# kongzhecn/OMG

Measured on NVIDIA H100. Metric: 1024^2 images/sec @30 steps, 2 concepts, higher is better.
Workload: dtype f16

## Files before the change

omg_b200/csrc/attn_tc.cu:

```cuda
#include <cuda_fp16.h>

#include <algorithm>
#include <math.h>
#include <stdlib.h>
#include <string.h>

#include "../../include/omg_b200.h"
#include "host_common.h"
#include "ptx.cuh"
#include "wgmma.cuh"

namespace omg {

constexpr int ATT_BQ = 128;
constexpr int ATT_BKV = 64;
constexpr int ATT_D = 64;
constexpr int ATT_Q_BYTES = ATT_BQ * ATT_D * 2;
constexpr int ATT_K_BYTES = ATT_BKV * ATT_D * 2;
constexpr int ATT_KV_STAGES = 4;
constexpr int ATT_THREADS = 256;
constexpr int ATT_SMEM = 1024 + ATT_Q_BYTES + ATT_KV_STAGES * 2 * ATT_K_BYTES + 256;

struct alignas(64) AttnParams {
    CUtensorMap q_map, k_map, v_map;
    __half* out;
    int out_ld;
    long long out_bs;
    int n_q, n_kv, heads;
    int q_col0, k_col0, v_col0, out_col0;
    int n_items;
    int out_b[OMG_ATTN_MAX_ITEMS], q_b[OMG_ATTN_MAX_ITEMS], k_b[OMG_ATTN_MAX_ITEMS], v_b[OMG_ATTN_MAX_ITEMS];
    float scale_log2;
    float out_weight;
    int accumulate;
    int causal;
};

__global__ void __launch_bounds__(ATT_THREADS, 2) attn_tc_kernel(const __grid_constant__ AttnParams p) {
    extern __shared__ uint8_t smem_raw[];
    uint8_t* smem = reinterpret_cast<uint8_t*>((reinterpret_cast<uintptr_t>(smem_raw) + 1023) & ~uintptr_t(1023));
    uint8_t* q_smem = smem;
    uint8_t* kv_smem = q_smem + ATT_Q_BYTES;
    uint64_t* q_full = reinterpret_cast<uint64_t*>(kv_smem + ATT_KV_STAGES * 2 * ATT_K_BYTES);
    uint64_t* kv_full = q_full + 1;
    uint64_t* kv_empty = kv_full + ATT_KV_STAGES;

    const int warp = threadIdx.x >> 5;
    const int lane = threadIdx.x & 31;
    const int slab = blockIdx.x, head = blockIdx.y, item = blockIdx.z;
    const int nkv = (p.n_kv + ATT_BKV - 1) / ATT_BKV;

    const int kb = p.k_b[item], vb = p.v_b[item];
    auto load_kv = [&](int jb) {
        const int st = jb % ATT_KV_STAGES;
        mbar_wait_nocall(&kv_empty[st], ((jb / ATT_KV_STAGES) & 1) ^ 1);
        uint8_t* kd = kv_smem + st * 2 * ATT_K_BYTES;
        mbar_arrive_expect_tx(&kv_full[st], 2 * ATT_K_BYTES);
        tma_load_3d(kd, &p.k_map, &kv_full[st], p.k_col0 + head * ATT_D, jb * ATT_BKV, kb);
        tma_load_3d(kd + ATT_K_BYTES, &p.v_map, &kv_full[st], p.v_col0 + head * ATT_D, jb * ATT_BKV, vb);
    };
    if (threadIdx.x == 0) {
        tma_prefetch_desc(&p.q_map);
        tma_prefetch_desc(&p.k_map);
        tma_prefetch_desc(&p.v_map);
        mbar_init(q_full, 1);
        for (int i = 0; i < ATT_KV_STAGES; ++i) {
            mbar_init(&kv_full[i], 1);
            mbar_init(&kv_empty[i], 2);
        }
        fence_barrier_init();
    }
    __syncthreads();
    griddep_launch_dependents();
    griddep_wait();
    if (threadIdx.x == 0) {
        mbar_arrive_expect_tx(q_full, ATT_Q_BYTES);
        tma_load_3d(q_smem, &p.q_map, q_full, p.q_col0 + head * ATT_D, slab * ATT_BQ, p.q_b[item]);
        for (int jb = 0; jb < ATT_KV_STAGES && jb < nkv; ++jb) load_kv(jb);
    }

    const int wg = warp >> 2, wi = warp & 3;
    const int g = lane >> 2, c = lane & 3;
    const int qrow0 = slab * ATT_BQ + wg * 64 + wi * 16 + g;
    const uint32_t q_addr = smem_u32(q_smem) + wg * (64 * 128);
    float o[32];
#pragma unroll
    for (int i = 0; i < 32; ++i) o[i] = 0.f;
    float m[2] = {-INFINITY, -INFINITY}, l[2] = {0.f, 0.f};
    mbar_wait_nocall(q_full, 0);
    for (int j = 0; j < nkv; ++j) {
        const int st = j % ATT_KV_STAGES;
        mbar_wait_nocall(&kv_full[st], (j / ATT_KV_STAGES) & 1);
        const uint32_t k_addr = smem_u32(kv_smem + st * 2 * ATT_K_BYTES);
        float s[32];
#pragma unroll
        for (int i = 0; i < 32; ++i) s[i] = 0.f;
        wgmma_fence();
#pragma unroll
        for (int k = 0; k < ATT_D / 16; ++k)
            wgmma_ss_n64(s, gmma_desc_sw128(q_addr + k * 32, 1024, 16), gmma_desc_sw128(k_addr + k * 32, 1024, 16), 1u);
        wgmma_commit();
        if (threadIdx.x == 0 && j >= 1 && j - 1 + ATT_KV_STAGES < nkv) load_kv(j - 1 + ATT_KV_STAGES);
        __syncwarp();
        wgmma_wait<0>();
        reg_fence(s);
        const int key0 = j * ATT_BKV + 2 * c;
        if ((j + 1) * ATT_BKV > p.n_kv || p.causal) {
#pragma unroll
            for (int J = 0; J < 8; ++J)
#pragma unroll
                for (int h = 0; h < 2; ++h)
#pragma unroll
                    for (int e = 0; e < 2; ++e) {
                        const int key = key0 + 8 * J + e;
                        if (key >= p.n_kv || (p.causal && key > qrow0 + 8 * h)) s[4 * J + 2 * h + e] = -INFINITY;
                    }
        }
        float mx[2] = {-INFINITY, -INFINITY};
#pragma unroll
        for (int J = 0; J < 8; ++J)
#pragma unroll
            for (int h = 0; h < 2; ++h) mx[h] = fmaxf(mx[h], fmaxf(s[4 * J + 2 * h], s[4 * J + 2 * h + 1]));
        float corr[2];
#pragma unroll
        for (int h = 0; h < 2; ++h) {
            mx[h] = fmaxf(mx[h], __shfl_xor_sync(0xffffffffu, mx[h], 1));
            mx[h] = fmaxf(mx[h], __shfl_xor_sync(0xffffffffu, mx[h], 2));
            const float m_new = fmaxf(m[h], mx[h] * p.scale_log2);
            corr[h] = fast_exp2(m[h] - m_new);
            m[h] = m_new;
            l[h] *= corr[h];
        }
#pragma unroll
        for (int J = 0; J < 8; ++J)
#pragma unroll
            for (int h = 0; h < 2; ++h) {
                o[4 * J + 2 * h] *= corr[h];
                o[4 * J + 2 * h + 1] *= corr[h];
            }
        uint32_t pa[4][4];
#pragma unroll
        for (int kk = 0; kk < 4; ++kk)
#pragma unroll
            for (int t = 0; t < 4; ++t) {
                const int h = t & 1, i0 = 8 * kk + 4 * (t >> 1) + 2 * h;
                const float p0 = fast_exp2(fmaf(s[i0], p.scale_log2, -m[h]));
                const float p1 = fast_exp2(fmaf(s[i0 + 1], p.scale_log2, -m[h]));
                l[h] += p0 + p1;
                pa[kk][t] = pack_half2(p0, p1);
            }
        const uint32_t v_addr = k_addr + ATT_K_BYTES;
        wgmma_fence();
#pragma unroll
        for (int kk = 0; kk < 4; ++kk)
            wgmma_rs_n64_tb(o, pa[kk], gmma_desc_sw128(v_addr + kk * 2048, 1024, 1024), 1u);
        wgmma_commit();
        wgmma_wait<0>();
        reg_fence(o);
        if ((threadIdx.x & 127) == 0) mbar_arrive(&kv_empty[st]);
    }

#pragma unroll
    for (int h = 0; h < 2; ++h) {
        l[h] += __shfl_xor_sync(0xffffffffu, l[h], 1);
        l[h] += __shfl_xor_sync(0xffffffffu, l[h], 2);
        const int qrow = qrow0 + 8 * h;
        if (qrow < p.n_q) {
            const float inv = p.out_weight / l[h];
            __half* op = p.out + (long long)p.out_b[item] * p.out_bs + (long long)qrow * p.out_ld + p.out_col0 +
                         head * ATT_D + 2 * c;
#pragma unroll
            for (int J = 0; J < 8; ++J) {
                float v0 = o[4 * J + 2 * h] * inv, v1 = o[4 * J + 2 * h + 1] * inv;
                __half2* dst = reinterpret_cast<__half2*>(op + 8 * J);
                if (p.accumulate) {
                    const float2 f = __half22float2(*dst);
                    v0 += f.x;
                    v1 += f.y;
                }
                *dst = __floats2half2_rn(v0, v1);
            }
        }
    }
}

static int make_attn_map(CUtensorMap* m, const void* ptr, int cols, int ld, int tokens, long long bs, int nb,
                         uint32_t box_rows) {
    const uint64_t dims[3] = {(uint64_t)cols, (uint64_t)tokens, (uint64_t)nb};
    const uint64_t strides[3] = {1, (uint64_t)ld, (uint64_t)bs};
    const uint32_t box[3] = {64, box_rows, 1};
    return make_tmap(m, CU_TENSOR_MAP_DATA_TYPE_FLOAT16, ptr, 3, dims, strides, box, CU_TENSOR_MAP_SWIZZLE_128B);
}

}

using namespace omg;

static int attention_impl(const omg_attn_desc* d, void* stream_) {
    cudaStream_t stream = reinterpret_cast<cudaStream_t>(stream_);
    OMG_CHECK(d != nullptr, "omg_attention: null descriptor");
    OMG_CHECK(d->head_dim == 64, "omg_attention: head_dim %d unsupported (SDXL uses 64)", d->head_dim);
    OMG_CHECK(d->n_items >= 1 && d->n_items <= OMG_ATTN_MAX_ITEMS, "omg_attention: n_items=%d out of range",
              d->n_items);
    OMG_CHECK(d->n_q >= 1 && d->n_kv >= 1 && d->heads >= 1, "omg_attention: empty problem");
    OMG_CHECK(d->q && d->k && d->v && d->out, "omg_attention: null pointer");
    OMG_CHECK(d->out_ld % 8 == 0 && d->out_col0 % 8 == 0 && d->out_bs % 8 == 0,
              "omg_attention: output must be 16 B aligned per row");
    if (check_head_windows("omg_attention", d->heads, d->head_dim, {d->q_col0, d->k_col0, d->v_col0, d->out_col0},
                           {d->q_ld, d->k_ld, d->v_ld, d->out_ld}))
        return 1;
    OMG_CHECK(!d->causal || (d->n_kv <= 128 && d->n_q <= 128), "omg_attention: causal masking is available for sequences of <= 128 tokens");
    static bool configured = false;
    if (!configured) {
        OMG_CUDA(cudaFuncSetAttribute(attn_tc_kernel, cudaFuncAttributeMaxDynamicSharedMemorySize, ATT_SMEM));
        configured = true;
    }
    AttnParams p;
    memset(&p, 0, sizeof(p));
    int max_qb = 0, max_kb = 0, max_vb = 0;
    for (int i = 0; i < d->n_items; ++i) {
        p.out_b[i] = d->out_b[i];
        p.q_b[i] = d->q_b[i];
        p.k_b[i] = d->k_b[i];
        p.v_b[i] = d->v_b[i];
        max_qb = d->q_b[i] > max_qb ? d->q_b[i] : max_qb;
        max_kb = d->k_b[i] > max_kb ? d->k_b[i] : max_kb;
        max_vb = d->v_b[i] > max_vb ? d->v_b[i] : max_vb;
        OMG_CHECK(d->out_b[i] >= 0 && d->q_b[i] >= 0 && d->k_b[i] >= 0 && d->v_b[i] >= 0,
                  "omg_attention: negative batch index in item %d", i);
    }
    const int cols = d->heads * 64;
    if (make_attn_map(&p.q_map, d->q, d->q_col0 + cols, d->q_ld, d->n_q, d->q_bs, max_qb + 1, ATT_BQ)) return 1;
    if (make_attn_map(&p.k_map, d->k, d->k_col0 + cols, d->k_ld, d->n_kv, d->k_bs, max_kb + 1, ATT_BKV)) return 1;
    if (make_attn_map(&p.v_map, d->v, d->v_col0 + cols, d->v_ld, d->n_kv, d->v_bs, max_vb + 1, ATT_BKV)) return 1;
    p.out = static_cast<__half*>(d->out);
    p.out_ld = d->out_ld;
    p.out_bs = d->out_bs;
    p.n_q = d->n_q;
    p.n_kv = d->n_kv;
    p.heads = d->heads;
    p.q_col0 = d->q_col0;
    p.k_col0 = d->k_col0;
    p.v_col0 = d->v_col0;
    p.out_col0 = d->out_col0;
    p.n_items = d->n_items;
    p.scale_log2 = d->scale * 1.4426950408889634f;
    p.out_weight = d->out_weight;
    p.accumulate = d->accumulate;
    p.causal = d->causal;
    dim3 grid((d->n_q + ATT_BQ - 1) / ATT_BQ, d->heads, d->n_items);
    OMG_CUDA(launch_pdl(attn_tc_kernel, grid, dim3(ATT_THREADS), ATT_SMEM, stream, p));
    return check_launch("attn_tc_kernel");
}

extern "C" int omg_attention(const omg_attn_desc* d, void* stream_) {
    const int rc = attention_impl(d, stream_);
    if (rc == 0 && ::omg::plan_recording()) {
        const omg_attn_desc c = *d;
        ::omg::plan_note([c](void* s) { return attention_impl(&c, s); });
    }
    return rc;
}
```

Measured before the change: 0.2027.

## Restructure attention into persistent warp-specialized kernel with pingpong softmax overlap

Rewrites the flash attention kernel as a persistent, warp-specialized design. A producer warp issues TMA loads for Q (double-buffered) and K/V tiles, and two consumer warpgroups alternate wgmma issue through turn barriers. The QK^T of the next block overlaps with PV and softmax of the current one. It also enlarges the KV block to 128, rebalances registers with setmaxnreg, and computes part of the exponentials with a polynomial exp2 to offload the SFU. This adds scheduling complexity, a grid of at most one CTA per SM, and slight numeric differences from the polynomial exp.

```diff
diff --git a/omg_b200/csrc/attn_tc.cu b/omg_b200/csrc/attn_tc.cu
--- a/omg_b200/csrc/attn_tc.cu
+++ b/omg_b200/csrc/attn_tc.cu
@@ -13,13 +13,14 @@
 namespace omg {
 
 constexpr int ATT_BQ = 128;
-constexpr int ATT_BKV = 64;
+constexpr int ATT_BKV = 128;
 constexpr int ATT_D = 64;
 constexpr int ATT_Q_BYTES = ATT_BQ * ATT_D * 2;
 constexpr int ATT_K_BYTES = ATT_BKV * ATT_D * 2;
 constexpr int ATT_KV_STAGES = 4;
-constexpr int ATT_THREADS = 256;
-constexpr int ATT_SMEM = 1024 + ATT_Q_BYTES + ATT_KV_STAGES * 2 * ATT_K_BYTES + 256;
+constexpr int ATT_THREADS = 384;
+constexpr int ATT_SMEM = 1024 + 2 * ATT_Q_BYTES + ATT_KV_STAGES * 2 * ATT_K_BYTES + 256;
+constexpr int ATT_POLY8 = 1;
 
 struct alignas(64) AttnParams {
     CUtensorMap q_map, k_map, v_map;
@@ -29,6 +30,7 @@
     int n_q, n_kv, heads;
     int q_col0, k_col0, v_col0, out_col0;
     int n_items;
+    int n_qt, n_tiles;
     int out_b[OMG_ATTN_MAX_ITEMS], q_b[OMG_ATTN_MAX_ITEMS], k_b[OMG_ATTN_MAX_ITEMS], v_b[OMG_ATTN_MAX_ITEMS];
     float scale_log2;
     float out_weight;
@@ -36,34 +38,40 @@
     int causal;
 };
 
-__global__ void __launch_bounds__(ATT_THREADS, 2) attn_tc_kernel(const __grid_constant__ AttnParams p) {
+__device__ __forceinline__ float poly_exp2(float x) {
+    x = fmaxf(x, -126.f);
+    const float t = __fadd_rd(x, 12582912.f);
+    const float f = x - (t - 12582912.f);
+    const float p = fmaf(fmaf(fmaf(0.07802452892065048f, f, 0.22606714069843292f), f, 0.6958335638046265f), f,
+                         0.9999251961708069f);
+    return __uint_as_float(__float_as_uint(p) + (__float_as_uint(t) << 23));
+}
+
+__global__ void __launch_bounds__(ATT_THREADS, 1) attn_tc_kernel(const __grid_constant__ AttnParams p) {
     extern __shared__ uint8_t smem_raw[];
     uint8_t* smem = reinterpret_cast<uint8_t*>((reinterpret_cast<uintptr_t>(smem_raw) + 1023) & ~uintptr_t(1023));
     uint8_t* q_smem = smem;
-    uint8_t* kv_smem = q_smem + ATT_Q_BYTES;
+    uint8_t* kv_smem = q_smem + 2 * ATT_Q_BYTES;
     uint64_t* q_full = reinterpret_cast<uint64_t*>(kv_smem + ATT_KV_STAGES * 2 * ATT_K_BYTES);
-    uint64_t* kv_full = q_full + 1;
+    uint64_t* q_empty = q_full + 2;
+    uint64_t* kv_full = q_empty + 2;
     uint64_t* kv_empty = kv_full + ATT_KV_STAGES;
+    uint64_t* turn_bar = kv_empty + ATT_KV_STAGES;
 
     const int warp = threadIdx.x >> 5;
     const int lane = threadIdx.x & 31;
-    const int slab = blockIdx.x, head = blockIdx.y, item = blockIdx.z;
     const int nkv = (p.n_kv + ATT_BKV - 1) / ATT_BKV;
-
-    const int kb = p.k_b[item], vb = p.v_b[item];
-    auto load_kv = [&](int jb) {
-        const int st = jb % ATT_KV_STAGES;
-        mbar_wait_nocall(&kv_empty[st], ((jb / ATT_KV_STAGES) & 1) ^ 1);
-        uint8_t* kd = kv_smem + st * 2 * ATT_K_BYTES;
-        mbar_arrive_expect_tx(&kv_full[st], 2 * ATT_K_BYTES);
-        tma_load_3d(kd, &p.k_map, &kv_full[st], p.k_col0 + head * ATT_D, jb * ATT_BKV, kb);
-        tma_load_3d(kd + ATT_K_BYTES, &p.v_map, &kv_full[st], p.v_col0 + head * ATT_D, jb * ATT_BKV, vb);
-    };
-    if (threadIdx.x == 0) {
+    const int per_item = p.n_qt * p.heads;
+
+    if (warp == 8 && lane == 0) {
         tma_prefetch_desc(&p.q_map);
         tma_prefetch_desc(&p.k_map);
         tma_prefetch_desc(&p.v_map);
-        mbar_init(q_full, 1);
+        for (int i = 0; i < 2; ++i) {
+            mbar_init(&q_full[i], 1);
+            mbar_init(&q_empty[i], 2);
+            mbar_init(&turn_bar[i], 1);
+        }
         for (int i = 0; i < ATT_KV_STAGES; ++i) {
             mbar_init(&kv_full[i], 1);
             mbar_init(&kv_empty[i], 2);
@@ -73,112 +81,204 @@
     __syncthreads();
     griddep_launch_dependents();
     griddep_wait();
-    if (threadIdx.x == 0) {
-        mbar_arrive_expect_tx(q_full, ATT_Q_BYTES);
-        tma_load_3d(q_smem, &p.q_map, q_full, p.q_col0 + head * ATT_D, slab * ATT_BQ, p.q_b[item]);
-        for (int jb = 0; jb < ATT_KV_STAGES && jb < nkv; ++jb) load_kv(jb);
-    }
-
+
+    if (warp >= 8) {
+        asm volatile("setmaxnreg.dec.sync.aligned.u32 40;");
+        if (warp == 8 && lane == 0) {
+            int kv_i = 0;
+            for (int t = blockIdx.x, qi = 0; t < p.n_tiles; t += gridDim.x, ++qi) {
+                const int item = t / per_item, head = (t % per_item) / p.n_qt, qt = t % p.n_qt;
+                const int qb = qi & 1;
+                mbar_wait_nocall(&q_empty[qb], ((qi >> 1) & 1) ^ 1);
+                mbar_arrive_expect_tx(&q_full[qb], ATT_Q_BYTES);
+                tma_load_3d(q_smem + qb * ATT_Q_BYTES, &p.q_map, &q_full[qb], p.q_col0 + head * ATT_D, qt * ATT_BQ,
+                            p.q_b[item]);
+                const int kb = p.k_b[item], vb = p.v_b[item];
+                for (int jb = 0; jb < nkv; ++jb, ++kv_i) {
+                    const int st = kv_i % ATT_KV_STAGES;
+                    mbar_wait_nocall(&kv_empty[st], ((kv_i / ATT_KV_STAGES) & 1) ^ 1);
+                    uint8_t* kd = kv_smem + st * 2 * ATT_K_BYTES;
+                    mbar_arrive_expect_tx(&kv_full[st], 2 * ATT_K_BYTES);
+                    tma_load_3d(kd, &p.k_map, &kv_full[st], p.k_col0 + head * ATT_D, jb * ATT_BKV, kb);
+                    tma_load_3d(kd + ATT_K_BYTES, &p.v_map, &kv_full[st], p.v_col0 + head * ATT_D, jb * ATT_BKV, vb);
+                }
+            }
+        }
+        return;
+    }
+
+    asm volatile("setmaxnreg.inc.sync.aligned.u32 232;");
     const int wg = warp >> 2, wi = warp & 3;
     const int g = lane >> 2, c = lane & 3;
-    const int qrow0 = slab * ATT_BQ + wg * 64 + wi * 16 + g;
-    const uint32_t q_addr = smem_u32(q_smem) + wg * (64 * 128);
+    const bool leader = (threadIdx.x & 127) == 0;
+    uint32_t turn_phase = wg == 0 ? 1u : 0u;
+    auto take_turn = [&]() {
+        mbar_wait_nocall(&turn_bar[wg], turn_phase);
+        turn_phase ^= 1;
+    };
+    auto pass_turn = [&]() {
+        if (leader) mbar_arrive(&turn_bar[wg ^ 1]);
+    };
+    int kv_i = 0;
     float o[32];
-#pragma unroll
-    for (int i = 0; i < 32; ++i) o[i] = 0.f;
-    float m[2] = {-INFINITY, -INFINITY}, l[2] = {0.f, 0.f};
-    mbar_wait_nocall(q_full, 0);
-    for (int j = 0; j < nkv; ++j) {
-        const int st = j % ATT_KV_STAGES;
-        mbar_wait_nocall(&kv_full[st], (j / ATT_KV_STAGES) & 1);
-        const uint32_t k_addr = smem_u32(kv_smem + st * 2 * ATT_K_BYTES);
-        float s[32];
-#pragma unroll
-        for (int i = 0; i < 32; ++i) s[i] = 0.f;
-        wgmma_fence();
-#pragma unroll
-        for (int k = 0; k < ATT_D / 16; ++k)
-            wgmma_ss_n64(s, gmma_desc_sw128(q_addr + k * 32, 1024, 16), gmma_desc_sw128(k_addr + k * 32, 1024, 16), 1u);
-        wgmma_commit();
-        if (threadIdx.x == 0 && j >= 1 && j - 1 + ATT_KV_STAGES < nkv) load_kv(j - 1 + ATT_KV_STAGES);
-        __syncwarp();
-        wgmma_wait<0>();
-        reg_fence(s);
-        const int key0 = j * ATT_BKV + 2 * c;
-        if ((j + 1) * ATT_BKV > p.n_kv || p.causal) {
+    uint32_t pa[8][4], pb[8][4];
+
+    for (int t = blockIdx.x, qi = 0; t < p.n_tiles; t += gridDim.x, ++qi) {
+        const int item = t / per_item, head = (t % per_item) / p.n_qt, qt = t % p.n_qt;
+        const int qrow0 = qt * ATT_BQ + wg * 64 + wi * 16 + g;
+        const int qb = qi & 1;
+        const uint32_t q_addr = smem_u32(q_smem + qb * ATT_Q_BYTES) + wg * (64 * 128);
+        float m[2] = {-INFINITY, -INFINITY}, l[2] = {0.f, 0.f};
+#pragma unroll
+        for (int i = 0; i < 32; ++i) o[i] = 0.f;
+
+        auto issue_qk = [&](float (&s)[64], int st) {
+            const uint32_t k_addr = smem_u32(kv_smem + st * 2 * ATT_K_BYTES);
+#pragma unroll
+            for (int k = 0; k < ATT_D / 16; ++k)
+                wgmma_ss_n128(s, gmma_desc_sw128(q_addr + k * 32, 1024, 16), gmma_desc_sw128(k_addr + k * 32, 1024, 16),
+                              k > 0 ? 1u : 0u);
+            wgmma_commit();
+        };
+        auto issue_pv = [&](int st, const uint32_t (&pc)[8][4]) {
+            const uint32_t v_addr = smem_u32(kv_smem + st * 2 * ATT_K_BYTES + ATT_K_BYTES);
+#pragma unroll
+            for (int kk = 0; kk < ATT_BKV / 16; ++kk)
+                wgmma_rs_n64_tb(o, pc[kk], gmma_desc_sw128(v_addr + kk * 2048, 1024, 1024), 1u);
+            wgmma_commit();
+        };
+        auto softmax = [&](float (&s)[64], int j, uint32_t (&pn)[8][4], float (&corr)[2]) {
+            const int key0 = j * ATT_BKV + 2 * c;
+            if ((j + 1) * ATT_BKV > p.n_kv || p.causal) {
+#pragma unroll
+                for (int J = 0; J < 16; ++J)
+#pragma unroll
+                    for (int h = 0; h < 2; ++h)
+#pragma unroll
+                        for (int e = 0; e < 2; ++e) {
+                            const int key = key0 + 8 * J + e;
+                            if (key >= p.n_kv || (p.causal && key > qrow0 + 8 * h)) s[4 * J + 2 * h + e] = -INFINITY;
+                        }
+            }
+            float mx[2] = {-INFINITY, -INFINITY};
+#pragma unroll
+            for (int J = 0; J < 16; ++J)
+#pragma unroll
+                for (int h = 0; h < 2; ++h) mx[h] = fmaxf(mx[h], fmaxf(s[4 * J + 2 * h], s[4 * J + 2 * h + 1]));
+#pragma unroll
+            for (int h = 0; h < 2; ++h) {
+                mx[h] = fmaxf(mx[h], __shfl_xor_sync(0xffffffffu, mx[h], 1));
+                mx[h] = fmaxf(mx[h], __shfl_xor_sync(0xffffffffu, mx[h], 2));
+                const float m_new = fmaxf(m[h], mx[h] * p.scale_log2);
+                corr[h] = fast_exp2(m[h] - m_new);
+                m[h] = m_new;
+                l[h] *= corr[h];
+            }
+#pragma unroll
+            for (int kk = 0; kk < 8; ++kk)
+#pragma unroll
+                for (int t2 = 0; t2 < 4; ++t2) {
+                    const int h = t2 & 1, i0 = 8 * kk + 4 * (t2 >> 1) + 2 * h;
+                    const float x0 = fmaf(s[i0], p.scale_log2, -m[h]), x1 = fmaf(s[i0 + 1], p.scale_log2, -m[h]);
+                    const bool poly = (4 * kk + t2) % 8 < ATT_POLY8;
+                    const float p0 = poly ? poly_exp2(x0) : fast_exp2(x0);
+                    const float p1 = poly ? poly_exp2(x1) : fast_exp2(x1);
+                    l[h] += p0 + p1;
+                    pn[kk][t2] = pack_half2(p0, p1);
+                }
+        };
+
+        mbar_wait_nocall(&q_full[qb], (qi >> 1) & 1);
+        int st = kv_i % ATT_KV_STAGES;
+        mbar_wait_nocall(&kv_full[st], (kv_i / ATT_KV_STAGES) & 1);
+        {
+            float s[64], corr[2];
+            take_turn();
+            wgmma_fence();
+            issue_qk(s, st);
+            pass_turn();
+            wgmma_wait<0>();
+            reg_fence(s);
+            softmax(s, 0, pa, corr);
+        }
+        auto step = [&](int j, const uint32_t (&pc)[8][4], uint32_t (&pn)[8][4]) {
+            const int st_prev = st;
+            ++kv_i;
+            st = kv_i % ATT_KV_STAGES;
+            mbar_wait_nocall(&kv_full[st], (kv_i / ATT_KV_STAGES) & 1);
+            take_turn();
+            float s[64], corr[2];
+            wgmma_fence();
+            issue_qk(s, st);
+            issue_pv(st_prev, pc);
+            pass_turn();
+            wgmma_wait<1>();
+            reg_fence(s);
+            softmax(s, j, pn, corr);
+            wgmma_wait<0>();
+            reg_fence(o);
+            if (leader) mbar_arrive(&kv_empty[st_prev]);
 #pragma unroll
             for (int J = 0; J < 8; ++J)
 #pragma unroll
+                for (int h = 0; h < 2; ++h) {
+                    o[4 * J + 2 * h] *= corr[h];
+                    o[4 * J + 2 * h + 1] *= corr[h];
+                }
+        };
+        __half* op[2];
+        __half2 prev[2][8];
+#pragma unroll
+        for (int h = 0; h < 2; ++h)
+            op[h] = p.out + (long long)p.out_b[item] * p.out_bs + (long long)(qrow0 + 8 * h) * p.out_ld + p.out_col0 +
+                    head * ATT_D + 2 * c;
+        auto last = [&](const uint32_t (&pc)[8][4]) {
+            if (leader) mbar_arrive(&q_empty[qb]);
+            take_turn();
+            wgmma_fence();
+            issue_pv(st, pc);
+            pass_turn();
+            if (p.accumulate)
+#pragma unroll
                 for (int h = 0; h < 2; ++h)
-#pragma unroll
-                    for (int e = 0; e < 2; ++e) {
-                        const int key = key0 + 8 * J + e;
-                        if (key >= p.n_kv || (p.causal && key > qrow0 + 8 * h)) s[4 * J + 2 * h + e] = -INFINITY;
+                    if (qrow0 + 8 * h < p.n_q)
+#pragma unroll
+                        for (int J = 0; J < 8; ++J) prev[h][J] = *reinterpret_cast<const __half2*>(op[h] + 8 * J);
+            wgmma_wait<0>();
+            reg_fence(o);
+            if (leader) mbar_arrive(&kv_empty[st]);
+            ++kv_i;
+        };
+        for (int j = 1;; j += 2) {
+            if (j >= nkv) {
+                last(pa);
+                break;
+            }
+            step(j, pa, pb);
+            if (j + 1 >= nkv) {
+                last(pb);
+                break;
+            }
+            step(j + 1, pb, pa);
+        }
+
+#pragma unroll
+        for (int h = 0; h < 2; ++h) {
+            l[h] += __shfl_xor_sync(0xffffffffu, l[h], 1);
+            l[h] += __shfl_xor_sync(0xffffffffu, l[h], 2);
+            if (qrow0 + 8 * h < p.n_q) {
+                const float inv = p.out_weight / l[h];
+#pragma unroll
+                for (int J = 0; J < 8; ++J) {
+                    float v0 = o[4 * J + 2 * h] * inv, v1 = o[4 * J + 2 * h + 1] * inv;
+                    __half2* dst = reinterpret_cast<__half2*>(op[h] + 8 * J);
+                    if (p.accumulate) {
+                        const float2 f = __half22float2(prev[h][J]);
+                        v0 += f.x;
+                        v1 += f.y;
                     }
-        }
-        float mx[2] = {-INFINITY, -INFINITY};
-#pragma unroll
-        for (int J = 0; J < 8; ++J)
-#pragma unroll
-            for (int h = 0; h < 2; ++h) mx[h] = fmaxf(mx[h], fmaxf(s[4 * J + 2 * h], s[4 * J + 2 * h + 1]));
-        float corr[2];
-#pragma unroll
-        for (int h = 0; h < 2; ++h) {
-            mx[h] = fmaxf(mx[h], __shfl_xor_sync(0xffffffffu, mx[h], 1));
-            mx[h] = fmaxf(mx[h], __shfl_xor_sync(0xffffffffu, mx[h], 2));
-            const float m_new = fmaxf(m[h], mx[h] * p.scale_log2);
-            corr[h] = fast_exp2(m[h] - m_new);
-            m[h] = m_new;
-            l[h] *= corr[h];
-        }
-#pragma unroll
-        for (int J = 0; J < 8; ++J)
-#pragma unroll
-            for (int h = 0; h < 2; ++h) {
-                o[4 * J + 2 * h] *= corr[h];
-                o[4 * J + 2 * h + 1] *= corr[h];
-            }
-        uint32_t pa[4][4];
-#pragma unroll
-        for (int kk = 0; kk < 4; ++kk)
-#pragma unroll
-            for (int t = 0; t < 4; ++t) {
-                const int h = t & 1, i0 = 8 * kk + 4 * (t >> 1) + 2 * h;
-                const float p0 = fast_exp2(fmaf(s[i0], p.scale_log2, -m[h]));
-                const float p1 = fast_exp2(fmaf(s[i0 + 1], p.scale_log2, -m[h]));
-                l[h] += p0 + p1;
-                pa[kk][t] = pack_half2(p0, p1);
-            }
-        const uint32_t v_addr = k_addr + ATT_K_BYTES;
-        wgmma_fence();
-#pragma unroll
-        for (int kk = 0; kk < 4; ++kk)
-            wgmma_rs_n64_tb(o, pa[kk], gmma_desc_sw128(v_addr + kk * 2048, 1024, 1024), 1u);
-        wgmma_commit();
-        wgmma_wait<0>();
-        reg_fence(o);
-        if ((threadIdx.x & 127) == 0) mbar_arrive(&kv_empty[st]);
-    }
-
-#pragma unroll
-    for (int h = 0; h < 2; ++h) {
-        l[h] += __shfl_xor_sync(0xffffffffu, l[h], 1);
-        l[h] += __shfl_xor_sync(0xffffffffu, l[h], 2);
-        const int qrow = qrow0 + 8 * h;
-        if (qrow < p.n_q) {
-            const float inv = p.out_weight / l[h];
-            __half* op = p.out + (long long)p.out_b[item] * p.out_bs + (long long)qrow * p.out_ld + p.out_col0 +
-                         head * ATT_D + 2 * c;
-#pragma unroll
-            for (int J = 0; J < 8; ++J) {
-                float v0 = o[4 * J + 2 * h] * inv, v1 = o[4 * J + 2 * h + 1] * inv;
-                __half2* dst = reinterpret_cast<__half2*>(op + 8 * J);
-                if (p.accumulate) {
-                    const float2 f = __half22float2(*dst);
-                    v0 += f.x;
-                    v1 += f.y;
+                    *dst = __floats2half2_rn(v0, v1);
                 }
-                *dst = __floats2half2_rn(v0, v1);
             }
         }
     }
@@ -211,8 +311,12 @@
         return 1;
     OMG_CHECK(!d->causal || (d->n_kv <= 128 && d->n_q <= 128), "omg_attention: causal masking is available for sequences of <= 128 tokens");
     static bool configured = false;
+    static int num_sms = 0;
     if (!configured) {
         OMG_CUDA(cudaFuncSetAttribute(attn_tc_kernel, cudaFuncAttributeMaxDynamicSharedMemorySize, ATT_SMEM));
+        int dev = 0;
+        OMG_CUDA(cudaGetDevice(&dev));
+        OMG_CUDA(cudaDeviceGetAttribute(&num_sms, cudaDevAttrMultiProcessorCount, dev));
         configured = true;
     }
     AttnParams p;
@@ -248,8 +352,9 @@
     p.out_weight = d->out_weight;
     p.accumulate = d->accumulate;
     p.causal = d->causal;
-    dim3 grid((d->n_q + ATT_BQ - 1) / ATT_BQ, d->heads, d->n_items);
-    OMG_CUDA(launch_pdl(attn_tc_kernel, grid, dim3(ATT_THREADS), ATT_SMEM, stream, p));
+    p.n_qt = (d->n_q + ATT_BQ - 1) / ATT_BQ;
+    p.n_tiles = p.n_qt * d->heads * d->n_items;
+    OMG_CUDA(launch_pdl(attn_tc_kernel, dim3(std::min(p.n_tiles, num_sms)), dim3(ATT_THREADS), ATT_SMEM, stream, p));
     return check_launch("attn_tc_kernel");
 }
 
```

Result: no change. 0.2044, median of 6 (+0.8%).
